# shanjiayao/PTT

Measured on AMD Instinct MI355X. Metric: tracklet frames/sec (hot path: PointNet++ SA stack + Point-Track-Transformer blocks), higher is better.
Workload: dtype f32

## Files before the change

### include/ptt_hip.h

```cpp
#ifndef PTT_HIP_H
#define PTT_HIP_H

#include <stddef.h>
#include <stdint.h>

#ifdef __cplusplus
extern "C" {
#endif

#define PTT_ABI_VERSION 39

enum {
    PTT_OK = 0,
    PTT_EINVAL = -1,
    PTT_EUNSUPPORTED = -2,
    PTT_ELAUNCH = -3,
    PTT_EWORKSPACE = -4
};

typedef void* ptt_stream_t;

int ptt_version(void);
const char* ptt_error_name(int code);
const char* ptt_last_error_string(void);

// ... 6 lines not shown
                 int B, int N, int C, int npoint, int32_t* idx_out, ptt_stream_t stream);

int ptt_gather_f32(const float* feat, const int32_t* idx, int B, int C, int N, int M,
                   float* out, ptt_stream_t stream);
int ptt_gather_grad_f32(const float* grad_out, const int32_t* idx, int B, int C, int N,
                        int M, float* grad_feat, ptt_stream_t stream);

int ptt_select_centres_f32(const float* xyz, const int32_t* idx, int B, int N, int M, float* new_xyz,
                           int64_t* idx64_out, ptt_stream_t stream);

int ptt_ball_query_f32(const float* new_xyz, const float* xyz, int B, int M, int N,
                       float radius, int nsample, int32_t* idx_out, ptt_stream_t stream);

int ptt_centres_ball_query_f32(const float* xyz, const int32_t* sel, int B, int N, int M, float radius, int nsample,
                               float* new_xyz, int64_t* idx64_out, int32_t* idx_out, ptt_stream_t stream);

int ptt_group_f32(const float* feat, const int32_t* idx, int B, int C, int N, int M,
                  int ns, float* out, ptt_stream_t stream);
int ptt_group_grad_f32(const float* grad_out, const int32_t* idx, int B, int C, int N,
                       int M, int ns, float* grad_feat, ptt_stream_t stream);

size_t ptt_scatter_add_det_workspace(int B, int N, int E);
int ptt_scatter_add_det_f32(const float* src, const int32_t* idx, int B, int C, int N, int E, float* out,
                            void* workspace, size_t workspace_bytes, ptt_stream_t stream);

int ptt_knn_f32(const float* xyz, int B, int N, int k, int32_t* idx_out,
                ptt_stream_t stream);
int ptt_knn_rel_f32(const float* xyz, int B, int N, int k, int32_t* idx_out, float* rel_out,
                    ptt_stream_t stream);

// ... 66 lines not shown
    int64_t feat_sb, feat_sc, feat_sn;
    float* out;
    int64_t out_sb, out_sc, out_sm;
    int B, N, M, nsample, C;
    float radius;
    int use_xyz;
    int normalize_xyz;
    int n_layers;
    ptt_sa_layer layers[PTT_SA_MAX_LAYERS];
    const float* l0_point_term;
    const float* l0_xyz_weight;
    int l0_channels;
    int l0_relu;
    void* compact_ws;
    size_t compact_ws_bytes;
} ptt_sa_desc;

int ptt_sa_fused_fwd_f32(const ptt_sa_desc* d, ptt_stream_t stream);
size_t ptt_sa_compact_workspace(int B, int M);

typedef struct ptt_xcorr_desc {
    const float* cos_t;
    const float* P;
    const float* w_sim;
    const float* scale0;
    const float* shift0;
    float* out;
    int64_t out_sb, out_sc, out_sn;
    float* sim_out;
    int B, Ns, Nt, C0;
// ... 500 lines not shown
```

### ptt_amd/_lib.py

```python
import ctypes
import os
import re
from ctypes import Structure, c_char_p, c_double, c_float, c_int, c_int32, c_int64, c_longlong, c_size_t, c_uint32, c_void_p

from .build import HEADER as HEADER_PATH, LIB as LIB_PATH


def _strip_comments(text):
    return re.sub(r"/\*.*?\*/|//[^\n]*", " ", text, flags=re.S)


def parse_defines(text):
    return {n: int(v) for n, v in re.findall(r"^[ \t]*#[ \t]*define[ \t]+(PTT_\w+)[ \t]+(-?\d+)[ \t]*$", _strip_comments(text), re.M)}


CTYPES = {"int": c_int, "int32_t": c_int32, "uint32_t": c_uint32, "int64_t": c_int64, "long long": c_longlong, "size_t": c_size_t,
          "float": c_float, "double": c_double, "ptt_stream_t": c_void_p}


def _ctype(decl, name, is_return=False):
    words = decl.replace("*", " * ").split()
    if not is_return and len(words) > 1 and words[-1] != "*":
        words.pop()
    if "*" in words:
# ... 170 lines not shown


class SaLayer(Structure):
    _fields_ = [("Wpacked", c_void_p), ("scale", c_void_p), ("shift", c_void_p),
                ("Cin", c_int), ("Cout", c_int), ("relu", c_int)]


class SaDesc(Structure):
    _fields_ = [("xyz", c_void_p), ("new_xyz", c_void_p), ("idx", c_void_p), ("feat", c_void_p),
                ("feat_sb", c_int64), ("feat_sc", c_int64), ("feat_sn", c_int64),
                ("out", c_void_p), ("out_sb", c_int64), ("out_sc", c_int64), ("out_sm", c_int64),
                ("B", c_int), ("N", c_int), ("M", c_int), ("nsample", c_int), ("C", c_int),
                ("radius", c_float), ("use_xyz", c_int), ("normalize_xyz", c_int), ("n_layers", c_int),
                ("layers", SaLayer * PTT_SA_MAX_LAYERS),
                ("l0_point_term", c_void_p), ("l0_xyz_weight", c_void_p), ("l0_channels", c_int), ("l0_relu", c_int),
                ("compact_ws", c_void_p), ("compact_ws_bytes", c_size_t)]


class XcorrDesc(Structure):
    _fields_ = [("cos_t", c_void_p), ("P", c_void_p), ("w_sim", c_void_p), ("scale0", c_void_p), ("shift0", c_void_p),
                ("out", c_void_p), ("out_sb", c_int64), ("out_sc", c_int64), ("out_sn", c_int64),
                ("sim_out", c_void_p),
                ("B", c_int), ("Ns", c_int), ("Nt", c_int), ("C0", c_int),
                ("n_layers", c_int), ("layers", SaLayer * PTT_SA_MAX_LAYERS),
                ("split", c_int32), ("out_sh", c_int64), ("search_feat", c_void_p), ("templ_feat", c_void_p),
                ("s_sb", c_int64), ("s_sn", c_int64), ("t_sb", c_int64), ("t_sn", c_int64), ("C", c_int), ("eps", c_float)]


class AttnDesc(Structure):
    _fields_ = [("xyz", c_void_p), ("rel", c_void_p), ("knn", c_void_p), ("qkv", c_void_p),
                ("Wd1p", c_void_p), ("Wd2p", c_void_p), ("bd2", c_void_p),
# ... 59 lines not shown
```

### ptt_amd/csrc/mfma_ops.hip

```cpp
#include <math.h>
#include <stdlib.h>
#include <string.h>
#include "common.h"
#include "mfma_common.h"

#ifndef PTT_PAIR_PF
#define PTT_PAIR_PF 1
#endif
#ifndef PTT_GATHER_BATCH
#define PTT_GATHER_BATCH 16
#endif
#ifndef PTT_SA_WAVES
#define PTT_SA_WAVES 2
#endif

namespace ptt {

#ifdef PTT_DEV
#define PTT_STAMP(i) do { if (p.dbg && threadIdx.x == 0 && blockIdx.x < 4096) p.dbg[blockIdx.x * 8 + (i)] = __builtin_readcyclecounter(); } while (0)
#else
#define PTT_STAMP(i) do { } while (0)
#endif

__device__ __forceinline__ void stagger_second_slot(int first_wave_blocks, int quanta) {
// ... 1260 lines not shown
            if (valid) tab.ndist()[g0 + lc] = nd;
        }
    }
    __syncthreads();
    if (t < 4) s_base[t] = s_cnt[t] ? atomicAdd(&tab.ws[t], s_cnt[t]) : 0;
    __syncthreads();
    for (int e = t; e < 32 * 32; e += 256) {
        const int lc = e >> 5, j = e & 31, k = s_cls[lc];
        if (k < 0 || j >= (4 << k)) continue;
        const int q = s_base[k] + s_pos[lc];
        tab.rows(k)[(size_t)q * (4 << k) + j] = s_row[lc][j < s_nd[lc] ? j : 0];
        if (j == 0) tab.list(k)[q] = g0 + lc;
    }
}

#ifndef PTT_SAL_WGS
#define PTT_SAL_WGS 1
#endif
#ifndef PTT_SAL_WAVES
#define PTT_SAL_WAVES 12
#endif

template <int ROWS>
struct SacTileT {
    static constexpr int LG = ROWS == 32 ? 3 : 4;
    static_assert(ROWS == 32 || ROWS == 64, "32- or 64-row tiles");
    int k, first, n;
    __device__ __forceinline__ static void count(const int32_t* ws, int total, int (&cnt)[4], int (&tiles)[4]) {
#pragma unroll
        for (int k = 0; k < 4; ++k) {
// ... 655 lines not shown
    return launch("rows_mlp_kernel", rows_mlp_kernel, dim3((rows + 31) / 32), dim3(256), lds, as_stream(stream), p);
}

extern "C" size_t ptt_sa_compact_workspace(int B, int M) {
    const long long T = (long long)(B > 0 ? B : 0) * (M > 0 ? M : 0);
    return SacTable::words((size_t)T) * sizeof(int32_t);
}

template <bool XYZ>
static int launch_ball_table(const ptt_sa_desc* d, SaParams& p, hipStream_t s) {
    if (d->compact_ws_bytes < ptt_sa_compact_workspace(d->B, d->M) || (reinterpret_cast<uintptr_t>(d->compact_ws) & 15))
        return fail(PTT_EWORKSPACE, "ptt_sa_fused_fwd_f32: compact_ws needs %zu bytes, 16-byte aligned (got %zu)",
                    ptt_sa_compact_workspace(d->B, d->M), d->compact_ws_bytes);
    const int total_centres = d->B * d->M;
    p.cws = static_cast<int32_t*>(d->compact_ws);
    hipLaunchKernelGGL(sa_compact_zero_kernel, dim3(1), dim3(64), 0, s, p.cws);
    if (int rc = check_launch("sa_compact_zero_kernel")) return rc;
    hipLaunchKernelGGL(sa_compact_kernel<XYZ>, dim3((total_centres + 31) / 32), dim3(256), 0, s, d->xyz, d->idx, d->N, d->M,
                       SacTable{p.cws, total_centres});
    return check_launch("sa_compact_kernel");
}

extern "C" int ptt_sa_fused_fwd_f32(const ptt_sa_desc* d, ptt_stream_t stream) {
    if (!d) return fail(PTT_EINVAL, "ptt_sa_fused_fwd_f32: null descriptor");
    if (d->B < 0 || d->N <= 0 || d->M < 0 || d->C < 0 || d->n_layers < 1 || d->n_layers > PTT_SA_MAX_LAYERS)
        return fail(PTT_EINVAL, "ptt_sa_fused_fwd_f32: B=%d N=%d M=%d C=%d layers=%d", d->B, d->N, d->M, d->C,
                    d->n_layers);
    if (d->nsample != 16 && d->nsample != 32 && d->nsample != 64)
        return fail(PTT_EUNSUPPORTED, "ptt_sa_fused_fwd_f32: nsample=%d (16, 32 and 64 are instantiated)", d->nsample);
    if (d->B == 0 || d->M == 0) return PTT_OK;
// ... 219 lines not shown
```

### ptt_amd/csrc/point_ops.hip

```cpp
#pragma clang fp contract(off)

#include <limits.h>
#include <stdlib.h>
#include "common.h"

namespace ptt {

__device__ __forceinline__ float sqdist3(float ax, float ay, float az, float bx, float by, float bz) {
    const float dx = ax - bx, dy = ay - by, dz = az - bz;
    return (dx * dx + dy * dy) + dz * dz;
}

__device__ __forceinline__ float knn_dist(float ax, float ay, float az, float bx, float by, float bz) {
    const float d = sqdist3(ax, ay, az, bx, by, bz);
    return d < __builtin_inff() ? d : 3.402823466e+38f;
}

__device__ __forceinline__ float lane_bcast(float v, int src_lane) {
    return __builtin_bit_cast(float, __builtin_amdgcn_readlane(__builtin_bit_cast(int, v), src_lane));
}

typedef float fps_f2 __attribute__((ext_vector_type(2)));


// ... 181 lines not shown
            PTT_FPS_ABL_CASE(1) PTT_FPS_ABL_CASE(2) PTT_FPS_ABL_CASE(3) PTT_FPS_ABL_CASE(4) PTT_FPS_ABL_CASE(8) PTT_FPS_ABL_CASE(12) PTT_FPS_ABL_CASE(15)
            PTT_FPS_ABL_CASE(16) PTT_FPS_ABL_CASE(32) PTT_FPS_ABL_CASE(47) PTT_FPS_ABL_CASE(7) PTT_FPS_ABL_CASE(24) PTT_FPS_ABL_CASE(40)
#undef PTT_FPS_ABL_CASE
        }
#endif
        hipLaunchKernelGGL((fps_kernel<T, P, true>), dim3(B), dim3(T), sel_bytes + (size_t)N * 12, s, xyz, N, npoint, idx);
        return check_launch("fps_kernel");
    }
    hipLaunchKernelGGL((fps_kernel<T, P, false>), dim3(B), dim3(T), sel_bytes, s, xyz, N, npoint, idx);
    return check_launch("fps_kernel");
}

template <int CPW>
__device__ __forceinline__ void ball_sweep(const float* __restrict__ pts, int N, float r2, int ns, const float (&cx)[CPW],
                                           const float (&cy)[CPW], const float (&cz)[CPW], int ncentres,
                                           int32_t* __restrict__ out0, int lane) {
    int cnt[CPW], first[CPW];
#pragma unroll
    for (int c = 0; c < CPW; ++c) { cnt[c] = (c < ncentres) ? 0 : ns; first[c] = 0; }
    for (int base = 0; base < N; base += 64) {
        const int k = base + lane;
        const bool in = k < N;
        float px = 0.f, py = 0.f, pz = 0.f;
        if (in) { px = pts[3 * k + 0]; py = pts[3 * k + 1]; pz = pts[3 * k + 2]; }
        bool active = false;
#pragma unroll
        for (int c = 0; c < CPW; ++c) {
            if (cnt[c] >= ns) continue;
            const float d = sqdist3(cx[c], cy[c], cz[c], px, py, pz);
            const bool hit = in && d < r2;
            const unsigned long long mask = __ballot(hit);
            if (mask != 0ull) {
                if (cnt[c] == 0) first[c] = base + (__ffsll((long long)mask) - 1);
                const int pos = cnt[c] + __popcll(mask & ((1ull << lane) - 1ull));
                if (hit && pos < ns) out0[(size_t)c * ns + pos] = k;
                cnt[c] += __popcll(mask);
            }
            active = active || cnt[c] < ns;
        }
        if (!active) break;
    }
#pragma unroll
    for (int c = 0; c < CPW; ++c) {
        if (c >= ncentres) break;
        const int fill = (cnt[c] > 0) ? first[c] : 0;
        for (int s = cnt[c] + lane; s < ns; s += 64) out0[(size_t)c * ns + s] = fill;
    }
}

template <int CPW>
__global__ __launch_bounds__(256) void ball_query_kernel(const float* __restrict__ new_xyz,
                                                         const float* __restrict__ xyz, int BM, int M, int N,
                                                         float r2, int ns, int32_t* __restrict__ idx_out) {
    const int centre = (blockIdx.x * 4 + (threadIdx.x >> 6)) * CPW;
    if (centre >= BM) return;
    const int lane = threadIdx.x & 63;
    const int b = centre / M;
    float cx[CPW], cy[CPW], cz[CPW];
    const int nc = min(CPW, BM - centre);
#pragma unroll
    for (int c = 0; c < CPW; ++c) {
        const int cc = centre + (c < nc ? c : 0);
        cx[c] = new_xyz[(size_t)cc * 3 + 0]; cy[c] = new_xyz[(size_t)cc * 3 + 1]; cz[c] = new_xyz[(size_t)cc * 3 + 2];
    }
    ball_sweep<CPW>(xyz + (size_t)b * N * 3, N, r2, ns, cx, cy, cz, nc, idx_out + (size_t)centre * ns, lane);
}

template <int CPW>
__global__ __launch_bounds__(256) void centres_ball_query_kernel(const float* __restrict__ xyz, const int32_t* __restrict__ sel,
                                                                 int BM, int M, int N, float r2, int ns,
                                                                 float* __restrict__ new_xyz, long long* __restrict__ idx64,
                                                                 int32_t* __restrict__ idx_out) {
    const int centre = (blockIdx.x * 4 + (threadIdx.x >> 6)) * CPW;
    if (centre >= BM) return;
    const int lane = threadIdx.x & 63;
    const int b = centre / M;
    const float* __restrict__ pts = xyz + (size_t)b * N * 3;
    float cx[CPW], cy[CPW], cz[CPW];
    const int nc = min(CPW, BM - centre);
#pragma unroll
    for (int c = 0; c < CPW; ++c) {
        const int cc = centre + (c < nc ? c : 0);
        const int n = sel ? sel[cc] : cc - b * M;
        cx[c] = pts[3 * n + 0]; cy[c] = pts[3 * n + 1]; cz[c] = pts[3 * n + 2];
        if (lane == 0 && c < nc) {
            new_xyz[(size_t)cc * 3 + 0] = cx[c]; new_xyz[(size_t)cc * 3 + 1] = cy[c]; new_xyz[(size_t)cc * 3 + 2] = cz[c];
            if (idx64) idx64[cc] = n;
        }
    }
    ball_sweep<CPW>(pts, N, r2, ns, cx, cy, cz, nc, idx_out + (size_t)centre * ns, lane);
}

__global__ void gather_kernel(const float* __restrict__ feat, const int32_t* __restrict__ idx, int C, int N, int M,
                              float* __restrict__ out, size_t total) {
    for (size_t e = (size_t)blockIdx.x * blockDim.x + threadIdx.x; e < total; e += (size_t)gridDim.x * blockDim.x) {
        const int j = (int)(e % M);
        const size_t bc = e / M;
        const int b = (int)(bc / C);
        out[e] = feat[bc * N + idx[(size_t)b * M + j]];
    }
}
__global__ void gather_grad_kernel(const float* __restrict__ go, const int32_t* __restrict__ idx, int C, int N, int M,
                                   float* __restrict__ gf, size_t total) {
    for (size_t e = (size_t)blockIdx.x * blockDim.x + threadIdx.x; e < total; e += (size_t)gridDim.x * blockDim.x) {
        const int j = (int)(e % M);
// ... 999 lines not shown
                       C, N, M, grad_feat, total);
    return check_launch("gather_grad_kernel");
}

extern "C" int ptt_group_f32(const float* feat, const int32_t* idx, int B, int C, int N, int M, int ns, float* out,
                             ptt_stream_t stream) {
    if (B < 0 || C < 0 || N <= 0 || M < 0 || ns < 0) return fail(PTT_EINVAL, "ptt_group_f32: bad sizes");
    const size_t total = (size_t)B * C * M * ns;
    if (total == 0) return PTT_OK;
    if (!feat || !idx || !out) return fail(PTT_EINVAL, "ptt_group_f32: null pointer");
    hipLaunchKernelGGL(group_kernel, dim3(grid_for(total, 256)), dim3(256), 0, as_stream(stream), feat, idx, C, N, M,
                       ns, out, total);
    return check_launch("group_kernel");
}

extern "C" int ptt_centres_ball_query_f32(const float* xyz, const int32_t* sel, int B, int N, int M, float radius, int nsample,
                                          float* new_xyz, int64_t* idx64_out, int32_t* idx_out, ptt_stream_t stream) {
    if (B < 0 || M < 0 || N <= 0 || nsample <= 0 || (!sel && M > N))
        return fail(PTT_EINVAL, "ptt_centres_ball_query_f32: B=%d M=%d N=%d nsample=%d", B, M, N, nsample);
    if (B == 0 || M == 0) return PTT_OK;
    if (!xyz || !new_xyz || !idx_out) return fail(PTT_EINVAL, "ptt_centres_ball_query_f32: null pointer");
    const int BM = B * M;
    const int cpw = ball_cpw(BM, M);
    if (cpw == 8)
        hipLaunchKernelGGL((centres_ball_query_kernel<8>), dim3((BM / 8 + 3) / 4), dim3(256), 0, as_stream(stream), xyz, sel, BM,
                           M, N, radius * radius, nsample, new_xyz, reinterpret_cast<long long*>(idx64_out), idx_out);
    else if (cpw == 4)
        hipLaunchKernelGGL((centres_ball_query_kernel<4>), dim3((BM / 4 + 3) / 4), dim3(256), 0, as_stream(stream), xyz, sel, BM,
                           M, N, radius * radius, nsample, new_xyz, reinterpret_cast<long long*>(idx64_out), idx_out);
    else
        hipLaunchKernelGGL((centres_ball_query_kernel<1>), dim3((BM + 3) / 4), dim3(256), 0, as_stream(stream), xyz, sel, BM, M,
                           N, radius * radius, nsample, new_xyz, reinterpret_cast<long long*>(idx64_out), idx_out);
    return check_launch("centres_ball_query_kernel");
}


extern "C" size_t ptt_ball_query_grid_workspace(int B, int N) {
    if (B <= 0 || N <= 0) return 0;
    return (size_t)B * grid_slice_ints(N) * sizeof(int32_t);
}

static int ball_query_grid_launch(const char* who, const float* xyz, const float* centres, const int32_t* sel, int sel_mode, int B, int N, int M,
                                  float radius, int nsample, float* new_xyz, int64_t* idx64, int32_t* idx_out, void* ws, size_t ws_bytes,
                                  ptt_stream_t stream) {
    if (B < 0 || M < 0 || N <= 0 || nsample <= 0) return fail(PTT_EINVAL, "%s: B=%d M=%d N=%d nsample=%d", who, B, M, N, nsample);
    if (B == 0 || M == 0) return PTT_OK;
    if (N > 131072) return fail(PTT_EUNSUPPORTED, "%s: N=%d (the hit bitmap of a wave lives in LDS: at most 131072 points)", who, N);
    if (!ws || ws_bytes < ptt_ball_query_grid_workspace(B, N) || (reinterpret_cast<uintptr_t>(ws) & 15))
// ... 159 lines not shown
```

### ptt_amd/models/__init__.py

```python
from typing import NamedTuple

import numpy as np
import torch

from .trackers import build_tracker


def build_network(model_cfg, num_class, dataset):
    return build_tracker(model_cfg=model_cfg, num_class=num_class, dataset=dataset)


def _to_device_f32(val, device):
    if isinstance(val, np.ndarray):
        if val.dtype.kind not in 'fiub':
            return None
        val = torch.from_numpy(np.ascontiguousarray(val))
    elif not isinstance(val, torch.Tensor):
        return None
    if val.is_complex():
        return None
    if val.device.type == 'cpu' and device.type == 'cuda' and val.numel() > 0:
        val = val.pin_memory()
    return val.to(device=device, dtype=torch.float32, non_blocking=True)

# ... 30 lines not shown
```

### ptt_amd/models/backbones_3d/pointnet2/pointnet2_modules.py

```python
import os
from typing import List

import torch
import torch.nn as nn
import torch.nn.functional as F

from .... import ops, train_ops
from ....param_cache import (DropsCachesOnModeChange, FoldedLayer, ParamCache, conv_bn_tensors, fold_conv_bn,
                             index_table)
from . import pointnet2_utils
from . import pytorch_utils as pt_utils

STREAM_COMPACT_MIN_BALLS = 2048
STREAM_COMPACT_MAX_POINTS = 1024
PRECISIONS = ('fp32', 'bf16x2')
SPLIT_STREAM_MIN_BALLS = 0


class PointnetSAModuleVotes(DropsCachesOnModeChange, nn.Module):
    def __init__(self, *, mlp: List[int], radius: float = None, nsample: int = None, bn: bool = True,
                 use_xyz: bool = True, normalize_xyz: bool = False, sample_uniformly: bool = False,
                 sample_method='fps'):
        super().__init__()
        self.radius = radius
# ... 129 lines not shown
            xyz = xyz.contiguous()
            inds, inds64, new_xyz, idx, self.centres_knn = ops.fps_ball_knn(xyz, npoint, self.radius, self.nsample, self.centres_knn_k)
            pre = (new_xyz, idx, inds64)
        prefix = inds is None and self.sample_method in ('rs', 'sequence')
        if pre is not None:
            pass
        elif prefix:
            inds64 = index_table(xyz.size(0), npoint, xyz.device, torch.int64)
        elif inds is None:
            inds = self._sample(xyz, features, npoint)
        else:
            assert inds.shape[1] == npoint
            inds = inds.to(torch.int32)

        xyz = xyz.contiguous()
        if pre is not None:
            new_xyz, idx, inds64 = pre
        elif prefix:
            new_xyz, _, idx = ops.centres_ball_query(xyz, None, npoint, self.radius, self.nsample)
        else:
            new_xyz, inds64, idx = ops.centres_ball_query(xyz, inds.contiguous(), npoint, self.radius, self.nsample)
        layers, hoist = self._fused_params(xyz.device)
        split = self.precision == 'bf16x2'
        if split and (hoist is None or features is None):
            ops.note_precision_fallback(self._name(), self._split_reason(features, hoist, layers, xyz.shape[0], npoint, False))
        if hoist is not None and features is not None:
            wf_packed, wx, c0, relu0 = hoist
            rows = features.transpose(1, 2)
            uniform = rows.stride(2) == 1 and rows.stride(0) == rows.shape[1] * rows.stride(1)
            term = ops.linear(rows if uniform else rows.contiguous(), wf_packed, c0, None, layers[0].shift, relu=False)
            B, M, ns = xyz.shape[0], npoint, self.nsample
            if (B * M * ns <= ops.ONE_FRAME_MAX_SA_ROWS and ns in (16, 32) and len(layers) == 3 and c0 % 4 == 0 and c0 >= 192):
                if split:
                    ops.note_precision_fallback(self._name(), 'a handful of frames: the one-frame row-job forms are fp32 only')
                L1, L2 = layers[1], layers[2]
                h = torch.empty((B * M * ns, L1.cout), dtype=torch.float32, device=xyz.device)
                ops.row_jobs([pt_utils.layer_job(L1, prologue=3, x=term, idx=idx, xyz=xyz, centres=new_xyz, wx=wx,
                                                 radius=self.radius, ns=ns, M=M, N=xyz.shape[1], normalize_xyz=self.normalize_xyz,
                                                 pro_relu=relu0, out=h)])
                pooled = torch.empty((B, M, L2.cout), dtype=torch.float32, device=xyz.device)
                ops.row_jobs([pt_utils.layer_job(L2, x=h, epilogue=2, ns=ns, M=M, out=pooled)])
                return new_xyz, pooled.transpose(1, 2), inds64
            compact_gated = bool(compact) and B * M >= STREAM_COMPACT_MIN_BALLS and xyz.shape[1] <= STREAM_COMPACT_MAX_POINTS
            if split:
                reason = self._split_reason(features, hoist, layers, B, M, compact_gated)
                if reason is None:
                    S = self._split_params(xyz.device)
                    new_features = ops.sa_stream_split(xyz, new_xyz, idx, (term, wx, relu0), S['w1s'], S['shift1'], S['w2s'],
                                                       S['shift2'], self.radius, self.normalize_xyz, relu2=S['relu2'])
                    return new_xyz, new_features, inds64
                ops.note_precision_fallback(self._name(), reason)
            new_features = ops.sa_fused_forward(xyz, new_xyz, idx, None, layers[1:], self.radius, True,
                                                self.normalize_xyz, point_major_out=True, l0=(term, wx, relu0),
                                                compact=compact_gated)
        else:
            new_features = ops.sa_fused_forward(xyz, new_xyz, idx, features, layers, self.radius,
                                                self.use_xyz, self.normalize_xyz, point_major_out=True,
                                                compact=features is None)
        return new_xyz, new_features, inds64

    def _forward_train(self, xyz, features, npoint, inds):
        if inds is None:
            inds = self._sample(xyz, features, npoint)
        else:
            assert inds.shape[1] == npoint
            inds = inds.to(torch.int32)
        hoist = (self.use_xyz and not self.sample_uniformly and self.nsample * npoint <= 16384
                 and train_ops.usable(self.mlp_module, xyz if features is None else features)
                 and self.mlp_module[0].conv.weight.shape[0] % 4 == 0)
# ... 17 lines not shown
```

### ptt_amd/models/backbones_3d/pointnet2_backbone.py

```python
from typing import List

import torch
import torch.nn as nn

from ... import graph_policy, ops, train_ops
from ...param_cache import ParamCache, index_table
from .pointnet2 import pointnet2_modules


class PointNet2BackboneLight(nn.Module):
    def __init__(self, model_cfg, input_channels, **kwargs):
        super().__init__()
        self.model_cfg = model_cfg
        input_channels -= 3
        self.num_points_each_layer = []
        self.SA_modules = nn.ModuleList()
        sa = self.model_cfg.SA_CONFIG
        for k in range(len(sa.RADIUS)):
            mlps = list(sa.MLPS[k])
            if k == 0:
                mlps[0] = input_channels
            self.SA_modules.append(pointnet2_modules.PointnetSAModuleVotes(
                radius=sa.RADIUS[k], nsample=sa.NSAMPLE[k], mlp=mlps,
                use_xyz=sa.get('USE_XYZ', True), normalize_xyz=sa.get('NORMALIZE_XYZ', True),
                sample_method=sa.SAMPLE_METHOD[k]))
            self.SA_modules[-1].precision = sa.get('PRECISION', 'fp32')
        self.cov_final = nn.Conv1d(256, 256, kernel_size=1)
        self.num_point_features = sa.MLPS[-1][-1]
        self._cov_cache = ParamCache()
        self.seed_knn = 16
        self.overlap_branches = True
        self._side_stream = None

    @staticmethod
    def _break_up_pc(pc):
        xyz = pc[..., 0:3].contiguous()
        features = pc[..., 3:].contiguous() if pc.size(-1) > 3 else None
        return xyz, features

    def _cov_final(self, features):
        if not features.is_cuda:
            return self.cov_final(features)
        if self.training:
            if features.dtype != torch.float32:
                return self.cov_final(features)
            return train_ops.rows_linear(self.cov_final, features.transpose(1, 2)).transpose(1, 2)
        if ops.autograd_recording(self.cov_final, features) or features.dtype != torch.float32:
# ... 42 lines not shown
            inds = inds0.gather(1, inds1).gather(1, inds2)
        if want_knn:
            return xyz, point_features, inds, knn
        return xyz, point_features, inds

    def sample(self, search_points, template_points):
        from .pointnet2 import pointnet2_utils
        sa = self.model_cfg.SA_CONFIG
        assert sa.SAMPLE_METHOD[0] == 'fps'
        return (pointnet2_utils.furthest_point_sample(search_points[..., 0:3].contiguous(), sa.NPOINTS_SEARCH[0]),
                pointnet2_utils.furthest_point_sample(template_points[..., 0:3].contiguous(), sa.NPOINTS_TEMPLATE[0]))

    def forward_branches(self, search_points, template_points, inds=None):
        sa = self.model_cfg.SA_CONFIG
        i_s, i_t = inds if inds is not None else (None, None)
        last = (len(self.SA_modules) - 1,) if (search_points.is_cuda and not self.training) else ()
        if not (self.overlap_branches and search_points.is_cuda and not self.training):
            r = self.branch_forward(search_points, sa.NPOINTS_SEARCH, i_s, want_knn=self.seed_knn, compact_levels=last)
            t_seeds, t_feats, t_inds = self.branch_forward(template_points, sa.NPOINTS_TEMPLATE, i_t)
        else:
            if self._side_stream is None or self._side_stream.device != search_points.device:
                self._side_stream = torch.cuda.Stream(device=search_points.device)
            main = torch.cuda.current_stream(search_points.device)
            side = graph_policy.branch(main, self._side_stream)
            with torch.cuda.stream(side):
                t_seeds, t_feats, t_inds = self.branch_forward(template_points, sa.NPOINTS_TEMPLATE, i_t)
            r = self.branch_forward(search_points, sa.NPOINTS_SEARCH, i_s, want_knn=self.seed_knn, compact_levels=last)
            graph_policy.join(main, side)
            if side is not main:
                for t in (t_seeds, t_feats, t_inds, template_points):
                    t.record_stream(main)
        s_seeds, s_feats, s_inds = r[:3]
        s_knn = r[3] if len(r) > 3 else None
        out = {'search_seeds': s_seeds, 'search_feats': s_feats, 'search_inds': s_inds,
               'template_seeds': t_seeds, 'template_feats': t_feats, 'template_inds': t_inds}
        if s_knn is not None:
            out['search_seeds_knn'] = s_knn
        return out

    def forward(self, batch_dict):
        batch_dict.update(self.forward_branches(batch_dict['search_points'], batch_dict['template_points'],
                                                batch_dict.pop('fps_inds', None)))
# ... 4 lines not shown
```

### ptt_amd/ops.py

```python
import contextlib
import ctypes
import math
import os

import torch

from . import _lib
from ._lib import AttnDesc, AttnSplitDesc, SaDesc, SaLayer, SaSplitDesc, XcorrDesc, XcorrSplitDesc


def _stream():
    return ctypes.c_void_p(torch.cuda.current_stream().cuda_stream)


_timing = None


def start_kernel_timing(names):
    global _timing
    _timing = {n: [] for n in names}


def stop_kernel_timing():
    global _timing
# ... 246 lines not shown
    _chk(new_xyz, "new_xyz", torch.float32, 3)
    _chk(xyz, "xyz", torch.float32, 3)
    B, M, _ = new_xyz.shape
    N = xyz.shape[1]
    out = torch.empty((B, M, int(nsample)), dtype=torch.int32, device=xyz.device)
    if GRID_BALL_QUERY_MIN_POINTS <= N <= 131072:
        ws, ws_arg = _workspace("ptt_ball_query_grid_workspace", xyz.device, B, N)
        _launch("ptt_ball_query_grid_f32", xyz.device, _ptr(new_xyz), _ptr(xyz), B, M, N, float(radius), int(nsample), _ptr(out), *ws_arg,
                timed='ptt_ball_query_f32')
    else:
        _launch("ptt_ball_query_f32", xyz.device, _ptr(new_xyz), _ptr(xyz), B, M, N, float(radius), int(nsample), _ptr(out),
                timed='ptt_ball_query_f32')
    return out


def centres_ball_query(xyz, sel, npoint, radius, nsample, want_idx64=True):
    _chk(xyz, "xyz", torch.float32, 3)
    B, N, _ = xyz.shape
    if sel is not None:
        _chk(sel, "sel", torch.int32, 2)
    M = int(npoint)
    new_xyz = torch.empty((B, M, 3), dtype=torch.float32, device=xyz.device)
    idx64 = torch.empty((B, M), dtype=torch.int64, device=xyz.device) if (want_idx64 and sel is not None) else None
    idx = torch.empty((B, M, int(nsample)), dtype=torch.int32, device=xyz.device)
    if GRID_BALL_QUERY_MIN_POINTS <= N <= 131072:
        ws, ws_arg = _workspace("ptt_ball_query_grid_workspace", xyz.device, B, N)
        _launch("ptt_centres_ball_query_grid_f32", xyz.device, _ptr(xyz), _ptr(sel), B, N, M, float(radius), int(nsample), _ptr(new_xyz), _ptr(idx64),
                _ptr(idx), *ws_arg, timed='ptt_ball_query_f32')
    else:
        _launch("ptt_centres_ball_query_f32", xyz.device, _ptr(xyz), _ptr(sel), B, N, M, float(radius), int(nsample), _ptr(new_xyz), _ptr(idx64),
                _ptr(idx), timed='ptt_ball_query_f32')
    return new_xyz, idx64, idx


def group_points(features, idx):
    _chk(features, "features", torch.float32, 3)
    _chk(idx, "idx", torch.int32, 3)
    B, C, N = features.shape
    _, M, ns = idx.shape
    out = torch.empty((B, C, M, ns), dtype=torch.float32, device=features.device)
    _launch("ptt_group_f32", features.device, _ptr(features), _ptr(idx), B, C, N, M, ns, _ptr(out))
    return out


def group_points_grad(grad_out, idx, N):
    _chk(grad_out, "grad_out", torch.float32, 4)
# ... 83 lines not shown
    _launch("ptt_linear_f32", x.device, _ptr(x2), rows, K, x2.stride(0) if rows > 1 else K, _ptr(wpacked), int(cout), _ptr(scale), _ptr(shift),
            1 if relu else 0, _ptr(r2), (r2.stride(0) if (r2 is not None and rows > 1) else int(cout)), _ptr(o2),
            o2.stride(0) if rows > 1 else int(cout), timed='ptt_linear_f32')
    return out


def _fill_layers(dst, layers):
    for L, (wp, sc, sh, cin, co, relu) in zip(dst, layers):
        L.Wpacked = wp.data_ptr()
        L.scale = sc.data_ptr() if sc is not None else None
        L.shift = sh.data_ptr() if sh is not None else None
        L.Cin, L.Cout, L.relu = int(cin), int(co), int(bool(relu))


def sa_fused_forward(xyz, new_xyz, idx, features, layers, radius, use_xyz=True, normalize_xyz=False,
                     point_major_out=True, l0=None, compact=False):
    _chk(xyz, "xyz", torch.float32, 3)
    _chk(new_xyz, "new_xyz", torch.float32, 3)
    _chk(idx, "idx", torch.int32, 3)
    B, N, _ = xyz.shape
    _, M, ns = idx.shape
    d = SaDesc()
    d.xyz, d.new_xyz, d.idx = xyz.data_ptr(), new_xyz.data_ptr(), idx.data_ptr()
    if features is not None:
        if not features.is_cuda or features.dtype != torch.float32 or features.dim() != 3:
            raise RuntimeError("features must be a (B,C,N) float32 device tensor")
        d.feat = features.data_ptr()
        d.feat_sb, d.feat_sc, d.feat_sn = features.stride()
        d.C = features.shape[1]
    else:
        d.feat, d.C = None, 0
# ... 14 lines not shown
        if features is not None:
            raise RuntimeError("with a hoisted layer 0 the point features are already inside l0[0]")
        _chk(term, "l0 point term", torch.float32, 3)
        _chk(wx, "l0 xyz weight", torch.float32, 2)
        if term.shape[0] != B or term.shape[1] != N or wx.shape[0] != 3 or wx.shape[1] != term.shape[2]:
            raise RuntimeError("l0 point term must be (B,N,C0) and the xyz weight (3,C0)")
        d.l0_point_term, d.l0_xyz_weight = term.data_ptr(), wx.data_ptr()
        d.l0_channels, d.l0_relu = term.shape[2], int(bool(l0_relu))
    if isinstance(compact, torch.Tensor):
        if not compact.is_cuda or compact.device != xyz.device or not compact.is_contiguous():
            raise RuntimeError("compact workspace must be a contiguous tensor on %s" % xyz.device)
        d.compact_ws, d.compact_ws_bytes = compact.data_ptr(), compact.numel() * compact.element_size()
    elif compact:
        ws, (_, d.compact_ws_bytes) = _workspace("ptt_sa_compact_workspace", xyz.device, B, M)
        d.compact_ws = ws.data_ptr()
    _launch("ptt_sa_fused_fwd_f32", xyz.device, ctypes.byref(d), timed='ptt_sa_fused_fwd_f32')
    return out


def sa_stream_split(xyz, new_xyz, idx, l0, w1s, shift1, w2s, shift2, radius, normalize_xyz=False, relu2=True, point_major_out=True,
                    out=None):
    _chk(xyz, "xyz", torch.float32, 3)
    _chk(new_xyz, "new_xyz", torch.float32, 3)
    _chk(idx, "idx", torch.int32, 3)
    B, N, _ = xyz.shape
    _, M, ns = idx.shape
    term, wx, l0_relu = l0
    _chk(term, "l0 point term", torch.float32, 3)
    _chk(wx, "l0 xyz weight", torch.float32, 2)
    if ns != 32 or tuple(term.shape) != (B, N, 128) or tuple(wx.shape) != (3, 128) or tuple(new_xyz.shape) != (B, M, 3):
# ... 1648 lines not shown
```

Measured before the change: 17410.

## Emit ball-query hit counts to build the SA compaction table directly

The ball query now records, for each centre, how many neighbours it actually found. A new sa_count_table_kernel uses these counts to build the compacted-ball bucket table in one pass, replacing the zero and compact kernels that re-derived distinct neighbours from xyz. The tracker compact policy also turns compaction on for SA levels 1 and 2 of both the search and template branches, not only the last search level. The risks are a prefix-count loop that rescans all earlier hits in every block, and bucketing by hit count instead of by distinct index, which only matches when the padding uses the first hit.

```diff
diff --git a/include/ptt_hip.h b/include/ptt_hip.h
--- a/include/ptt_hip.h
+++ b/include/ptt_hip.h
@@ -8,7 +8,7 @@
 extern "C" {
 #endif
 
-#define PTT_ABI_VERSION 39
+#define PTT_ABI_VERSION 40
 
 enum {
     PTT_OK = 0,
@@ -45,6 +45,8 @@
 
 int ptt_centres_ball_query_f32(const float* xyz, const int32_t* sel, int B, int N, int M, float radius, int nsample,
                                float* new_xyz, int64_t* idx64_out, int32_t* idx_out, ptt_stream_t stream);
+int ptt_centres_ball_query_hits_f32(const float* xyz, const int32_t* sel, int B, int N, int M, float radius, int nsample,
+                                    float* new_xyz, int64_t* idx64_out, int32_t* idx_out, int32_t* hits_out, ptt_stream_t stream);
 
 int ptt_group_f32(const float* feat, const int32_t* idx, int B, int C, int N, int M,
                   int ns, float* out, ptt_stream_t stream);
@@ -141,6 +143,7 @@
     int l0_relu;
     void* compact_ws;
     size_t compact_ws_bytes;
+    const int32_t* hits;
 } ptt_sa_desc;
 
 int ptt_sa_fused_fwd_f32(const ptt_sa_desc* d, ptt_stream_t stream);
diff --git a/ptt_amd/_lib.py b/ptt_amd/_lib.py
--- a/ptt_amd/_lib.py
+++ b/ptt_amd/_lib.py
@@ -208,7 +208,7 @@
                 ("radius", c_float), ("use_xyz", c_int), ("normalize_xyz", c_int), ("n_layers", c_int),
                 ("layers", SaLayer * PTT_SA_MAX_LAYERS),
                 ("l0_point_term", c_void_p), ("l0_xyz_weight", c_void_p), ("l0_channels", c_int), ("l0_relu", c_int),
-                ("compact_ws", c_void_p), ("compact_ws_bytes", c_size_t)]
+                ("compact_ws", c_void_p), ("compact_ws_bytes", c_size_t), ("hits", c_void_p)]
 
 
 class XcorrDesc(Structure):
diff --git a/ptt_amd/csrc/mfma_ops.hip b/ptt_amd/csrc/mfma_ops.hip
--- a/ptt_amd/csrc/mfma_ops.hip
+++ b/ptt_amd/csrc/mfma_ops.hip
@@ -1298,6 +1298,63 @@
     }
 }
 
+__global__ __launch_bounds__(256) void sa_count_table_kernel(const int32_t* __restrict__ hits, const int32_t* __restrict__ idx,
+                                                             SacTable tab) {
+    __shared__ int s_gt[4][3];
+    __shared__ int s_cls[32], s_pos[32], s_nd[32];
+    const int t = threadIdx.x, lane = t & 63, w = t >> 6;
+    const int g0 = blockIdx.x * 32, T = tab.T;
+    int gt4 = 0, gt8 = 0, gt16 = 0;
+    if ((reinterpret_cast<uintptr_t>(hits) & 15) == 0) {
+        const int4* h4 = reinterpret_cast<const int4*>(hits);
+#pragma unroll 4
+        for (int i = t; i < g0 / 4; i += 256) {
+            const int4 v = h4[i];
+            gt4 += (v.x > 4) + (v.y > 4) + (v.z > 4) + (v.w > 4);
+            gt8 += (v.x > 8) + (v.y > 8) + (v.z > 8) + (v.w > 8);
+            gt16 += (v.x > 16) + (v.y > 16) + (v.z > 16) + (v.w > 16);
+        }
+    } else {
+#pragma unroll 4
+        for (int i = t; i < g0; i += 256) {
+            const int v = hits[i];
+            gt4 += v > 4; gt8 += v > 8; gt16 += v > 16;
+        }
+    }
+#pragma unroll
+    for (int o = 32; o > 0; o >>= 1) {
+        gt4 += __shfl_xor(gt4, o); gt8 += __shfl_xor(gt8, o); gt16 += __shfl_xor(gt16, o);
+    }
+    if (lane == 0) { s_gt[w][0] = gt4; s_gt[w][1] = gt8; s_gt[w][2] = gt16; }
+    __syncthreads();
+    if (w == 0) {
+        const int a4 = s_gt[0][0] + s_gt[1][0] + s_gt[2][0] + s_gt[3][0];
+        const int a8 = s_gt[0][1] + s_gt[1][1] + s_gt[2][1] + s_gt[3][1];
+        const int a16 = s_gt[0][2] + s_gt[1][2] + s_gt[2][2] + s_gt[3][2];
+        const int base[4] = {g0 - a4, a4 - a8, a8 - a16, a16};
+        const int g = g0 + lane;
+        const bool valid = lane < 32 && g < T;
+        const int nd = valid ? min(max(hits[g], 1), 32) : 1;
+        const int k = nd <= 4 ? 0 : nd <= 8 ? 1 : nd <= 16 ? 2 : 3;
+        int pos = 0, tot[4];
+#pragma unroll
+        for (int c = 0; c < 4; ++c) {
+            const unsigned long long m = __ballot(valid && k == c);
+            if (k == c) pos = base[c] + __popcll(m & ((1ull << lane) - 1ull));
+            tot[c] = base[c] + __popcll(m);
+        }
+        if (lane < 32) { s_cls[lane] = valid ? k : -1; s_pos[lane] = pos; s_nd[lane] = nd; }
+        if (valid) { tab.ndist()[g] = nd; tab.list(k)[pos] = g; }
+        if (blockIdx.x == gridDim.x - 1 && lane < 4) tab.ws[lane] = lane == 0 ? tot[0] : lane == 1 ? tot[1] : lane == 2 ? tot[2] : tot[3];
+    }
+    __syncthreads();
+    for (int e = t; e < 32 * 32; e += 256) {
+        const int lc = e >> 5, j = e & 31, k = s_cls[lc];
+        if (k < 0 || j >= (4 << k)) continue;
+        tab.rows(k)[(size_t)s_pos[lc] * (4 << k) + j] = idx[(size_t)(g0 + lc) * 32 + (j < s_nd[lc] ? j : 0)];
+    }
+}
+
 #ifndef PTT_SAL_WGS
 #define PTT_SAL_WGS 1
 #endif
@@ -1983,6 +2040,13 @@
                     ptt_sa_compact_workspace(d->B, d->M), d->compact_ws_bytes);
     const int total_centres = d->B * d->M;
     p.cws = static_cast<int32_t*>(d->compact_ws);
+    if constexpr (!XYZ) {
+        if (d->hits) {
+            hipLaunchKernelGGL(sa_count_table_kernel, dim3((total_centres + 31) / 32), dim3(256), 0, s, d->hits, d->idx,
+                               SacTable{p.cws, total_centres});
+            return check_launch("sa_count_table_kernel");
+        }
+    }
     hipLaunchKernelGGL(sa_compact_zero_kernel, dim3(1), dim3(64), 0, s, p.cws);
     if (int rc = check_launch("sa_compact_zero_kernel")) return rc;
     hipLaunchKernelGGL(sa_compact_kernel<XYZ>, dim3((total_centres + 31) / 32), dim3(256), 0, s, d->xyz, d->idx, d->N, d->M,
diff --git a/ptt_amd/csrc/point_ops.hip b/ptt_amd/csrc/point_ops.hip
--- a/ptt_amd/csrc/point_ops.hip
+++ b/ptt_amd/csrc/point_ops.hip
@@ -219,7 +219,7 @@
 template <int CPW>
 __device__ __forceinline__ void ball_sweep(const float* __restrict__ pts, int N, float r2, int ns, const float (&cx)[CPW],
                                            const float (&cy)[CPW], const float (&cz)[CPW], int ncentres,
-                                           int32_t* __restrict__ out0, int lane) {
+                                           int32_t* __restrict__ out0, int lane, int32_t* __restrict__ hits0 = nullptr) {
     int cnt[CPW], first[CPW];
 #pragma unroll
     for (int c = 0; c < CPW; ++c) { cnt[c] = (c < ncentres) ? 0 : ns; first[c] = 0; }
@@ -250,6 +250,7 @@
         if (c >= ncentres) break;
         const int fill = (cnt[c] > 0) ? first[c] : 0;
         for (int s = cnt[c] + lane; s < ns; s += 64) out0[(size_t)c * ns + s] = fill;
+        if (hits0 && lane == 0) hits0[c] = max(1, min(cnt[c], ns));
     }
 }
 
@@ -275,7 +276,7 @@
 __global__ __launch_bounds__(256) void centres_ball_query_kernel(const float* __restrict__ xyz, const int32_t* __restrict__ sel,
                                                                  int BM, int M, int N, float r2, int ns,
                                                                  float* __restrict__ new_xyz, long long* __restrict__ idx64,
-                                                                 int32_t* __restrict__ idx_out) {
+                                                                 int32_t* __restrict__ idx_out, int32_t* __restrict__ hits) {
     const int centre = (blockIdx.x * 4 + (threadIdx.x >> 6)) * CPW;
     if (centre >= BM) return;
     const int lane = threadIdx.x & 63;
@@ -293,7 +294,7 @@
             if (idx64) idx64[cc] = n;
         }
     }
-    ball_sweep<CPW>(pts, N, r2, ns, cx, cy, cz, nc, idx_out + (size_t)centre * ns, lane);
+    ball_sweep<CPW>(pts, N, r2, ns, cx, cy, cz, nc, idx_out + (size_t)centre * ns, lane, hits ? hits + centre : nullptr);
 }
 
 __global__ void gather_kernel(const float* __restrict__ feat, const int32_t* __restrict__ idx, int C, int N, int M,
@@ -1323,24 +1324,38 @@
     return check_launch("group_kernel");
 }
 
-extern "C" int ptt_centres_ball_query_f32(const float* xyz, const int32_t* sel, int B, int N, int M, float radius, int nsample,
-                                          float* new_xyz, int64_t* idx64_out, int32_t* idx_out, ptt_stream_t stream) {
+static int centres_ball_query_launch(const char* who, const float* xyz, const int32_t* sel, int B, int N, int M, float radius,
+                                     int nsample, float* new_xyz, int64_t* idx64_out, int32_t* idx_out, int32_t* hits_out,
+                                     ptt_stream_t stream) {
     if (B < 0 || M < 0 || N <= 0 || nsample <= 0 || (!sel && M > N))
-        return fail(PTT_EINVAL, "ptt_centres_ball_query_f32: B=%d M=%d N=%d nsample=%d", B, M, N, nsample);
+        return fail(PTT_EINVAL, "%s: B=%d M=%d N=%d nsample=%d", who, B, M, N, nsample);
     if (B == 0 || M == 0) return PTT_OK;
-    if (!xyz || !new_xyz || !idx_out) return fail(PTT_EINVAL, "ptt_centres_ball_query_f32: null pointer");
+    if (!xyz || !new_xyz || !idx_out) return fail(PTT_EINVAL, "%s: null pointer", who);
     const int BM = B * M;
     const int cpw = ball_cpw(BM, M);
     if (cpw == 8)
         hipLaunchKernelGGL((centres_ball_query_kernel<8>), dim3((BM / 8 + 3) / 4), dim3(256), 0, as_stream(stream), xyz, sel, BM,
-                           M, N, radius * radius, nsample, new_xyz, reinterpret_cast<long long*>(idx64_out), idx_out);
+                           M, N, radius * radius, nsample, new_xyz, reinterpret_cast<long long*>(idx64_out), idx_out, hits_out);
     else if (cpw == 4)
         hipLaunchKernelGGL((centres_ball_query_kernel<4>), dim3((BM / 4 + 3) / 4), dim3(256), 0, as_stream(stream), xyz, sel, BM,
-                           M, N, radius * radius, nsample, new_xyz, reinterpret_cast<long long*>(idx64_out), idx_out);
+                           M, N, radius * radius, nsample, new_xyz, reinterpret_cast<long long*>(idx64_out), idx_out, hits_out);
     else
         hipLaunchKernelGGL((centres_ball_query_kernel<1>), dim3((BM + 3) / 4), dim3(256), 0, as_stream(stream), xyz, sel, BM, M,
-                           N, radius * radius, nsample, new_xyz, reinterpret_cast<long long*>(idx64_out), idx_out);
+                           N, radius * radius, nsample, new_xyz, reinterpret_cast<long long*>(idx64_out), idx_out, hits_out);
     return check_launch("centres_ball_query_kernel");
+}
+
+extern "C" int ptt_centres_ball_query_f32(const float* xyz, const int32_t* sel, int B, int N, int M, float radius, int nsample,
+                                          float* new_xyz, int64_t* idx64_out, int32_t* idx_out, ptt_stream_t stream) {
+    return centres_ball_query_launch("ptt_centres_ball_query_f32", xyz, sel, B, N, M, radius, nsample, new_xyz, idx64_out, idx_out,
+                                     nullptr, stream);
+}
+
+extern "C" int ptt_centres_ball_query_hits_f32(const float* xyz, const int32_t* sel, int B, int N, int M, float radius, int nsample,
+                                               float* new_xyz, int64_t* idx64_out, int32_t* idx_out, int32_t* hits_out,
+                                               ptt_stream_t stream) {
+    return centres_ball_query_launch("ptt_centres_ball_query_hits_f32", xyz, sel, B, N, M, radius, nsample, new_xyz, idx64_out,
+                                     idx_out, hits_out, stream);
 }
 
 
diff --git a/ptt_amd/models/__init__.py b/ptt_amd/models/__init__.py
--- a/ptt_amd/models/__init__.py
+++ b/ptt_amd/models/__init__.py
@@ -3,11 +3,16 @@
 import numpy as np
 import torch
 
+from .backbones_3d.pointnet2_backbone import TRACKER_COMPACT_POLICY, PointNet2BackboneLight
 from .trackers import build_tracker
 
 
 def build_network(model_cfg, num_class, dataset):
-    return build_tracker(model_cfg=model_cfg, num_class=num_class, dataset=dataset)
+    model = build_tracker(model_cfg=model_cfg, num_class=num_class, dataset=dataset)
+    backbone = getattr(model, 'backbone_3d', None)
+    if isinstance(backbone, PointNet2BackboneLight):
+        backbone.compact_policy = {k: tuple(v) for k, v in TRACKER_COMPACT_POLICY.items()}
+    return model
 
 
 def _to_device_f32(val, device):
diff --git a/ptt_amd/models/backbones_3d/pointnet2/pointnet2_modules.py b/ptt_amd/models/backbones_3d/pointnet2/pointnet2_modules.py
--- a/ptt_amd/models/backbones_3d/pointnet2/pointnet2_modules.py
+++ b/ptt_amd/models/backbones_3d/pointnet2/pointnet2_modules.py
@@ -167,8 +167,16 @@
             inds = inds.to(torch.int32)
 
         xyz = xyz.contiguous()
+        compact_gated = (bool(compact) and features is not None and xyz.shape[0] * npoint >= STREAM_COMPACT_MIN_BALLS
+                         and xyz.shape[1] <= STREAM_COMPACT_MAX_POINTS)
+        hits = None
         if pre is not None:
             new_xyz, idx, inds64 = pre
+        elif compact_gated:
+            new_xyz, i64, idx, hits = ops.centres_ball_query(xyz, None if prefix else inds.contiguous(), npoint, self.radius,
+                                                             self.nsample, want_hits=True)
+            if not prefix:
+                inds64 = i64
         elif prefix:
             new_xyz, _, idx = ops.centres_ball_query(xyz, None, npoint, self.radius, self.nsample)
         else:
@@ -194,7 +202,6 @@
                 pooled = torch.empty((B, M, L2.cout), dtype=torch.float32, device=xyz.device)
                 ops.row_jobs([pt_utils.layer_job(L2, x=h, epilogue=2, ns=ns, M=M, out=pooled)])
                 return new_xyz, pooled.transpose(1, 2), inds64
-            compact_gated = bool(compact) and B * M >= STREAM_COMPACT_MIN_BALLS and xyz.shape[1] <= STREAM_COMPACT_MAX_POINTS
             if split:
                 reason = self._split_reason(features, hoist, layers, B, M, compact_gated)
                 if reason is None:
@@ -205,7 +212,7 @@
                 ops.note_precision_fallback(self._name(), reason)
             new_features = ops.sa_fused_forward(xyz, new_xyz, idx, None, layers[1:], self.radius, True,
                                                 self.normalize_xyz, point_major_out=True, l0=(term, wx, relu0),
-                                                compact=compact_gated)
+                                                compact=compact_gated, hits=hits if compact_gated else None)
         else:
             new_features = ops.sa_fused_forward(xyz, new_xyz, idx, features, layers, self.radius,
                                                 self.use_xyz, self.normalize_xyz, point_major_out=True,
diff --git a/ptt_amd/models/backbones_3d/pointnet2_backbone.py b/ptt_amd/models/backbones_3d/pointnet2_backbone.py
--- a/ptt_amd/models/backbones_3d/pointnet2_backbone.py
+++ b/ptt_amd/models/backbones_3d/pointnet2_backbone.py
@@ -6,6 +6,9 @@
 from ... import graph_policy, ops, train_ops
 from ...param_cache import ParamCache, index_table
 from .pointnet2 import pointnet2_modules
+
+
+TRACKER_COMPACT_POLICY = {'search': (1, 2), 'template': (1, 2)}
 
 
 class PointNet2BackboneLight(nn.Module):
@@ -31,6 +34,7 @@
         self.seed_knn = 16
         self.overlap_branches = True
         self._side_stream = None
+        self.compact_policy = {'search': (len(self.SA_modules) - 1,), 'template': ()}
 
     @staticmethod
     def _break_up_pc(pc):
@@ -103,18 +107,20 @@
     def forward_branches(self, search_points, template_points, inds=None):
         sa = self.model_cfg.SA_CONFIG
         i_s, i_t = inds if inds is not None else (None, None)
-        last = (len(self.SA_modules) - 1,) if (search_points.is_cuda and not self.training) else ()
+        on = search_points.is_cuda and not self.training
+        c_s = tuple(self.compact_policy.get('search', ())) if on else ()
+        c_t = tuple(self.compact_policy.get('template', ())) if on else ()
         if not (self.overlap_branches and search_points.is_cuda and not self.training):
-            r = self.branch_forward(search_points, sa.NPOINTS_SEARCH, i_s, want_knn=self.seed_knn, compact_levels=last)
-            t_seeds, t_feats, t_inds = self.branch_forward(template_points, sa.NPOINTS_TEMPLATE, i_t)
+            r = self.branch_forward(search_points, sa.NPOINTS_SEARCH, i_s, want_knn=self.seed_knn, compact_levels=c_s)
+            t_seeds, t_feats, t_inds = self.branch_forward(template_points, sa.NPOINTS_TEMPLATE, i_t, compact_levels=c_t)
         else:
             if self._side_stream is None or self._side_stream.device != search_points.device:
                 self._side_stream = torch.cuda.Stream(device=search_points.device)
             main = torch.cuda.current_stream(search_points.device)
             side = graph_policy.branch(main, self._side_stream)
             with torch.cuda.stream(side):
-                t_seeds, t_feats, t_inds = self.branch_forward(template_points, sa.NPOINTS_TEMPLATE, i_t)
-            r = self.branch_forward(search_points, sa.NPOINTS_SEARCH, i_s, want_knn=self.seed_knn, compact_levels=last)
+                t_seeds, t_feats, t_inds = self.branch_forward(template_points, sa.NPOINTS_TEMPLATE, i_t, compact_levels=c_t)
+            r = self.branch_forward(search_points, sa.NPOINTS_SEARCH, i_s, want_knn=self.seed_knn, compact_levels=c_s)
             graph_policy.join(main, side)
             if side is not main:
                 for t in (t_seeds, t_feats, t_inds, template_points):
diff --git a/ptt_amd/ops.py b/ptt_amd/ops.py
--- a/ptt_amd/ops.py
+++ b/ptt_amd/ops.py
@@ -284,7 +284,7 @@
     return out
 
 
-def centres_ball_query(xyz, sel, npoint, radius, nsample, want_idx64=True):
+def centres_ball_query(xyz, sel, npoint, radius, nsample, want_idx64=True, want_hits=False):
     _chk(xyz, "xyz", torch.float32, 3)
     B, N, _ = xyz.shape
     if sel is not None:
@@ -293,13 +293,20 @@
     new_xyz = torch.empty((B, M, 3), dtype=torch.float32, device=xyz.device)
     idx64 = torch.empty((B, M), dtype=torch.int64, device=xyz.device) if (want_idx64 and sel is not None) else None
     idx = torch.empty((B, M, int(nsample)), dtype=torch.int32, device=xyz.device)
+    hits = None
     if GRID_BALL_QUERY_MIN_POINTS <= N <= 131072:
         ws, ws_arg = _workspace("ptt_ball_query_grid_workspace", xyz.device, B, N)
         _launch("ptt_centres_ball_query_grid_f32", xyz.device, _ptr(xyz), _ptr(sel), B, N, M, float(radius), int(nsample), _ptr(new_xyz), _ptr(idx64),
                 _ptr(idx), *ws_arg, timed='ptt_ball_query_f32')
+    elif want_hits:
+        hits = torch.empty((B, M), dtype=torch.int32, device=xyz.device)
+        _launch("ptt_centres_ball_query_hits_f32", xyz.device, _ptr(xyz), _ptr(sel), B, N, M, float(radius), int(nsample), _ptr(new_xyz),
+                _ptr(idx64), _ptr(idx), _ptr(hits), timed='ptt_ball_query_f32')
     else:
         _launch("ptt_centres_ball_query_f32", xyz.device, _ptr(xyz), _ptr(sel), B, N, M, float(radius), int(nsample), _ptr(new_xyz), _ptr(idx64),
                 _ptr(idx), timed='ptt_ball_query_f32')
+    if want_hits:
+        return new_xyz, idx64, idx, hits
     return new_xyz, idx64, idx
 
 
@@ -413,7 +420,7 @@
 
 
 def sa_fused_forward(xyz, new_xyz, idx, features, layers, radius, use_xyz=True, normalize_xyz=False,
-                     point_major_out=True, l0=None, compact=False):
+                     point_major_out=True, l0=None, compact=False, hits=None):
     _chk(xyz, "xyz", torch.float32, 3)
     _chk(new_xyz, "new_xyz", torch.float32, 3)
     _chk(idx, "idx", torch.int32, 3)
@@ -458,6 +465,11 @@
     elif compact:
         ws, (_, d.compact_ws_bytes) = _workspace("ptt_sa_compact_workspace", xyz.device, B, M)
         d.compact_ws = ws.data_ptr()
+    if hits is not None and d.compact_ws:
+        _chk(hits, "hits", torch.int32, 2)
+        if tuple(hits.shape) != (B, M) or not hits.is_contiguous() or hits.device != xyz.device:
+            raise RuntimeError("hits must be a contiguous (B,M) int32 tensor on %s" % xyz.device)
+        d.hits = hits.data_ptr()
     _launch("ptt_sa_fused_fwd_f32", xyz.device, ctypes.byref(d), timed='ptt_sa_fused_fwd_f32')
     return out
 
```

Result: no change. 17420 (median of 2 runs) (+0.0%).
